# montyhall/bot7

Hardware: AMD Instinct MI355X
Metric: EI candidates scored/sec at N=2048,d=32 (higher is better)
Workload: dtype f64

## Files before the change

bot7_amd/build.py:

```python
import concurrent.futures
import os
import subprocess
import sys

HERE = os.path.dirname(os.path.abspath(__file__))
ROOT = os.path.dirname(HERE)
CSRC = os.path.join(HERE, "csrc")
BUILD = os.path.join(HERE, "_build")
OUT = os.path.join(HERE, "libbot7hip.so")
SOURCES = ["context.hip", "grid_api.hip", "gp_api.hip", "nominate.hip", "blr_api.hip", "sobol.hip", "covar.hip", "potrf.hip", "potrf_persist.hip", "posterior.hip", "score.hip", "extras.hip", "comm.hip", "group.hip", "blr_small.hip", "gp_small.hip", "kpost_small.hip", "batch.hip", "mes.hip", "rff.hip", "slice.hip", "refine.hip", "kg.hip", "ehvi.hip", "trust_region.hip", "ehvi3.hip", "blr_ts.hip", "ts_hvi.hip", "ts_feas.hip", "ts_refine.hip"]
DIAG_ONLY_SOURCES = ["nll_small.hip"]
DIAG_OUT = os.path.join(ROOT, "tools", "_build", "libbot7hip_diag.so")
HEADERS = [os.path.join(CSRC, "b7_internal.h"), os.path.join(CSRC, "gemm_f64.h"), os.path.join(CSRC, "potrf_diag.h"), os.path.join(CSRC, "comm_rccl.h"), os.path.join(CSRC, "ksx_exp.h"), os.path.join(CSRC, "ksx_walk.h"), os.path.join(CSRC, "exp_table.h"), os.path.join(CSRC, "mes_math.h"), os.path.join(CSRC, "logei_math.h"), os.path.join(CSRC, "ehvi_math.h"), os.path.join(CSRC, "counter_rng.h"), os.path.join(CSRC, "gp_small_body.h"), os.path.join(CSRC, "post_ring_layout.h"),
           os.path.join(ROOT, "include", "bot7hip.h")]
HIPCC = os.environ.get("HIPCC", "/opt/rocm/bin/hipcc")
FLAGS = ["-O3", "-std=c++17", "-fPIC", "--offload-arch=gfx950", "-fno-fast-math", "-Wall",
         "-I" + os.path.join(ROOT, "include"), "-I" + CSRC, "-I/opt/rocm/include"]


def _stale(target, deps):
    if not os.path.exists(target):
        return True
    t = os.path.getmtime(target)
    return any(os.path.getmtime(d) > t for d in deps)


EXTRA_FLAGS = {"covar.hip": ["-mllvm", "-amdgpu-mfma-vgpr-form"], "batch.hip": ["-mllvm", "-amdgpu-mfma-vgpr-form"],
               "rff.hip": ["-mllvm", "-amdgpu-mfma-vgpr-form"],
               "ts_refine.hip": ["-mllvm", "-amdgpu-mfma-vgpr-form"],
               "kg.hip": ["-mllvm", "-amdgpu-mfma-vgpr-form"],
               "slice.hip": ["-mllvm", "-disable-machine-licm"]}


def _compile(src, diag=False):
    obj = os.path.join(BUILD, ("diag_" if diag else "") + src.replace(".hip", ".o"))
    path = os.path.join(CSRC, src)
    if _stale(obj, [path] + HEADERS + [os.path.abspath(__file__)]):
        subprocess.check_call([HIPCC] + FLAGS + EXTRA_FLAGS.get(src, []) + (["-DB7_DIAG"] if diag else []) + ["-c", path, "-o", obj])
        return obj, True
    return obj, False


def _mentions_diag(src):
    return "B7_DIAG" in open(os.path.join(CSRC, src)).read()


def build_diag(verbose=False):
    build()
    os.makedirs(os.path.dirname(DIAG_OUT), exist_ok=True)
    todo = [s for s in SOURCES if _mentions_diag(s)] + DIAG_ONLY_SOURCES
    with concurrent.futures.ThreadPoolExecutor(max_workers=min(8, len(todo))) as ex:
        res = dict(zip(todo, ex.map(lambda s: _compile(s, True), todo)))
    objs = [res[s][0] if s in res else os.path.join(BUILD, s.replace(".hip", ".o")) for s in SOURCES + DIAG_ONLY_SOURCES]
    if any(ch for _, ch in res.values()) or _stale(DIAG_OUT, objs):
        subprocess.check_call([HIPCC, "-shared", "-fPIC", "--offload-arch=gfx950", "-o", DIAG_OUT] + objs +
                              ["-ldl", "-Wl,-rpath,/opt/rocm/lib", "-Wl,--no-undefined", "-Wl,-Bsymbolic"])
        if verbose:
            print("built", DIAG_OUT)
    return DIAG_OUT


def posterior_isa():
    out = os.path.join(BUILD, "posterior.s")
    path = os.path.join(CSRC, "posterior.hip")
    if _stale(out, [path] + HEADERS + [os.path.abspath(__file__)]):
        subprocess.check_call([HIPCC] + [f for f in FLAGS if f != "-fPIC"] + ["-S", "--cuda-device-only", "-Wno-unused-command-line-argument",
                                                                            path, "-o", out])
    return out


def check_agpr_discipline():
    import re
    text = open(posterior_isa()).read()
    found = {}
    for m in re.finditer(r"^(_ZN\S*post_kernel_w4(?:ILi(\d)E|tILi\d+ELi\d+E)\S*):[^\n]*\n(.*?)\n\s*s_endpgm", text, flags=re.S | re.M):
        nj = int(m.group(2)) if m.group(2) else 16
        ntiles = 32 if nj == 16 else 8 * nj
        in_asm, stats, bad = False, {"mfma": 0, "mfma_from_zero": 0, "acc_reads": 0, "scratch": 0}, []
        for line in m.group(3).split("\n"):
            code = line.split(";")[0]
            if "ASMSTART" in line:
                in_asm = True
                continue
            if "ASMEND" in line:
                in_asm = False
                continue
            if in_asm:
                stats["mfma"] += "v_mfma_f64_16x16x4_f64" in code
                stats["mfma_from_zero"] += bool(re.search(r"v_mfma_f64_16x16x4_f64 a\[[^\]]*\], v\[[^\]]*\], v\[[^\]]*\], 0\s*$", code))
                stats["acc_reads"] += "v_accvgpr_read_b32" in code
            else:
                if re.search(r"(?<![A-Za-z0-9_.])a(\[|\d)", code):
                    bad.append(line.strip())
                if nj == 16 and re.search(r"\bm0\b", code):
                    bad.append(line.strip())
                stats["scratch"] += "scratch_" in code
        if bad or stats["scratch"] or stats["mfma_from_zero"] != ntiles or stats["acc_reads"] != 8 * ntiles:
            raise RuntimeError("post_kernel_w4<%d>: AGPR discipline broken: %r, compiler-generated AGPR uses: %r"
                               % (nj, stats, bad[:5]))
        found[nj] = stats
    if not {2, 4} <= set(found):
        raise RuntimeError("post_kernel_w4<2> and <4> expected in the ISA of posterior.hip, found %r" % sorted(found))
    return found


def build_post_probe():
    src = os.path.join(ROOT, "tools", "post_probe.hip")
    out = os.path.join(ROOT, "tools", "_build", "post_probe")
    os.makedirs(os.path.dirname(out), exist_ok=True)
    if _stale(out, [src, os.path.join(ROOT, "tools", "post_kernel_w8.h"), os.path.join(CSRC, "posterior.hip")] + HEADERS):
        subprocess.check_call([HIPCC, "--offload-arch=gfx950", "-O3", "-std=c++17", "-fno-fast-math", "-Wno-unused-value",
                               "-DB7_POST_NO_LAUNCHERS", "-I" + os.path.join(ROOT, "include"), "-I" + CSRC,
                               "-I/opt/rocm/include", "-o", out, src, "-Wl,-rpath,/opt/rocm/lib"])
    return out


def build(force=False, verbose=False):
    os.makedirs(BUILD, exist_ok=True)
    if force:
        for f in os.listdir(BUILD):
            os.remove(os.path.join(BUILD, f))
    with concurrent.futures.ThreadPoolExecutor(max_workers=min(8, len(SOURCES) + 2)) as ex:
        isa = ex.submit(check_agpr_discipline)
        probe = ex.submit(build_post_probe)
        results = list(ex.map(_compile, SOURCES))
        isa.result()
        probe.result()
    objs = [o for o, _ in results]
    if any(changed for _, changed in results) or _stale(OUT, objs):
        subprocess.check_call([HIPCC, "-shared", "-fPIC", "--offload-arch=gfx950", "-o", OUT] + objs +
                              ["-ldl", "-Wl,-rpath,/opt/rocm/lib", "-Wl,--no-undefined", "-Wl,-Bsymbolic"])
        if verbose:
            print("built", OUT)
    return OUT

# ... 6 lines not shown
```

bot7_amd/csrc/b7_internal.h:

```cpp
#pragma once
#include <hip/hip_runtime.h>
#include <stddef.h>
#include <stdint.h>

#include <map>
#include <string>
#include <vector>

#include "bot7hip.h"

constexpr int B7_NPAD = 128;
constexpr int B7_PANEL = 64;
constexpr int B7_PERSIST_NMAX = 4096;
constexpr int B7_MROWS = 256;
constexpr int B7_MAX_D = 96;

constexpr int B7_TAB_VAL = 0;
constexpr int B7_TAB_IDX = 1;
constexpr int B7_TAB_STATUS = 2;
constexpr int B7_TAB_ROWS = 3;
constexpr int B7_TAB_ROW0 = 4;
constexpr int B7_TAB_W = B7_TAB_ROW0 + B7_MAX_D;
constexpr int B7_MAX_WORLD = 64;

// ... 105 lines not shown
  double amp = 0, noise = 0, mean = 0;
  b7_gp_opts opts;
  int kernel = B7_KERNEL_ARDSE;
  DevBuf xobs;
  DevBuf w;
  DevBuf zsc;
  DevBuf zss;
  DevBuf K;
  DevBuf L;
  DevBuf Linv;
  DevBuf W;
  DevBuf dinv;
  DevBuf alpha;
  DevBuf resid;
  DevBuf atmp;
  DevBuf info;
  DevBuf ybuf;

  bool predicted = false;
  int64_t Mpred = 0;
  DevBuf mu;
  DevBuf var;
  DevBuf acc;
  bool acc_valid = false;
  int spin_us = 500;
  bool npad_small = true;
  bool potrf_small = true;
  bool blr_small = true;
  double fmin_scalar = 0.0;
  bool acc_fresh = false;
  int acc_kind = 0;
  DevBuf ks;
  size_t ks_bytes = (size_t)4 << 30;
  int diag_variant = 1;
  int inverse_inline = 1;
  PinnedBlock *pinned = nullptr, *pinned_dev = nullptr;
  std::vector<double> net_host;
  PinBuf pin_blr;
  PinBuf pin_eval;
  PinBuf pin_nll;
  PinBuf pin_slice;
  DevBuf slice_state;
  DevBuf slice_trace;
  int slice_trace_rpc = 0;
  int slice_trace_C = 0, slice_trace_D = 0;
  bool fmin_staged = false;
  bool potrf_attrs_set = false;
  bool linv_done = false;
  int potrf_sched = 3;
  int syrk_small = 1;
  int potrf_defer = 1;
  int potrf_group = 2;
  struct JobList { DevBuf buf; int n = 0; };
  std::map<int, JobList> pjobs_cache;
  DevBuf pstamps;
  int pjobs_nb = 0, pjobs_n = 0;
  DevBuf bhyp, bw, bzsc, bzss, bK, bL, bdinv, bflags, binfo, bresid, bterms, bLinv, balpha, bmu, bvar;
  bool persist_attr_set = false, persist_stamps = false;
  int persist_helpers = 0;
  int persist_aborts = 0;
  int nll_small = 1;
  bool kpost_small = true;
  bool fit_small = true;
  int persist_fault = -1;
  int potrf_sched_saved = 0;
  DevBuf part;
// ... 434 lines not shown
```

bot7_amd/csrc/context.hip:

```cpp
#include <stdarg.h>
#include <stdio.h>
#include <stdlib.h>
#include <string.h>

#include "b7_internal.h"

static thread_local std::string g_create_err;

int b7_fail(b7_ctx *c, int code, const char *fmt, ...) {
  char buf[512];
  va_list ap;
  va_start(ap, fmt);
  vsnprintf(buf, sizeof(buf), fmt, ap);
  va_end(ap);
  if (c)
    c->err = buf;
  else
    g_create_err = buf;
  return code;
}

int b7_ensure(b7_ctx *c, DevBuf &b, size_t bytes) {
  if (bytes == 0) bytes = 16;
  if (b.cap >= bytes) return B7_OK;
// ... 133 lines not shown
  if (const char *pv = getenv("B7_TS_FEAS_ONEPASS")) c->ts_feas_onepass = atoi(pv) ? 1 : 0;
#endif
  e = hipStreamCreateWithFlags(&c->stream, hipStreamNonBlocking);
  if (e == hipSuccess) e = hipEventCreateWithFlags(&c->ev_fit, hipEventDisableTiming);
  if (e == hipSuccess) e = hipHostMalloc((void **)&c->pinned, B7_PINNED_BYTES, hipHostMallocMapped);
  if (e == hipSuccess) e = hipHostGetDevicePointer((void **)&c->pinned_dev, c->pinned, 0);
  if (e != hipSuccess) {
    if (c->pinned) (void)hipHostFree(c->pinned);
    if (c->stream) (void)hipStreamDestroy(c->stream);
    delete c;
    return b7_fail(nullptr, B7_ERR_HIP, "stream / pinned result block creation: %s", hipGetErrorString(e));
  }
  if (b7_ensure(c, c->scratch, B7_SCRATCH_BYTES) != B7_OK) {
    g_create_err = c->err;
    b7_destroy(c);
    return B7_ERR_NOMEM;
  }
  *out = c;
  return B7_OK;
}

void b7_destroy(b7_ctx *c) {
  if (!c) return;
  (void)hipSetDevice(c->device);
  (void)hipStreamSynchronize(c->stream);
  (void)b7_comm_destroy(c);
  DevBuf *all[] = {&c->grid[0], &c->grid[1], &c->xobs, &c->w,     &c->zsc,  &c->zss,     &c->K,      &c->L,
                   &c->Linv,    &c->W,       &c->dinv, &c->alpha, &c->resid, &c->info,   &c->ybuf,   &c->mu,
                   &c->var,     &c->acc,     &c->ks,   &c->part,  &c->scratch, &c->tmpgrid, &c->tmpmu, &c->tmpvar, &c->fant, &c->feat, &c->netbuf, &c->atmp, &c->slots, &c->pstamps,
                   &c->bhyp, &c->bw, &c->bzsc, &c->bzss, &c->bK, &c->bL, &c->bdinv, &c->bflags, &c->binfo, &c->bresid, &c->bterms,
                   &c->bLinv, &c->balpha, &c->bmu, &c->bvar, &c->ticket, &c->bel, &c->belvec, &c->ystar, &c->mes_ticket, &c->mes_user,
                   &c->ts_paths, &c->ts_draw, &c->ts_work, &c->ts_user, &c->ts_ref_ws, &c->ts_ref_trace, &c->ts_ref_user, &c->slice_trace, &c->slice_state, &c->refine_ws, &c->refine_trace, &c->refine_user,
                   &c->feas, &c->feas_stage, &c->kg, &c->kgvec, &c->kg_slopes, &c->kg_user,
                   &c->ts_hvi, &c->ts_hvi_t, &c->ts_hvi_user, &c->ts_feas, &c->ts_feas_user, &c->post, &c->ehvi_front, &c->ehvi_user, &c->ehvi3_front, &c->ehvi3_table, &c->ehvi3_user};
  for (auto &kv : c->pjobs_cache) b7_release(kv.second.buf);
  for (DevBuf *b : all) b7_release(*b);
  if (c->tev_init)
    for (int i = 0; i < B7_MAX_TIMERS; ++i) {
      (void)hipEventDestroy(c->tev[i][0]);
      (void)hipEventDestroy(c->tev[i][1]);
    }
  resolve_phases(c);
  if (c->pinned) (void)hipHostFree(c->pinned);
  for (PinBuf *b : {&c->pin_eval, &c->pin_blr, &c->pin_nll, &c->pin_bel, &c->pin_slice, &c->pin_kg})
    if (b->host) (void)hipHostFree(b->host);
  if (c->tab_host) (void)hipHostFree(c->tab_host);
  for (hipEvent_t e : c->free_events) (void)hipEventDestroy(e);
  if (c->phase_e0) (void)hipEventDestroy(c->phase_e0);
  if (c->ev_fit) (void)hipEventDestroy(c->ev_fit);
  for (hipEvent_t e : c->ev_feas)
    if (e) (void)hipEventDestroy(e);
  for (hipEvent_t e : c->ev_ehvi)
    if (e) (void)hipEventDestroy(e);
  for (hipEvent_t e : c->ev_ts_feas)
    if (e) (void)hipEventDestroy(e);
  (void)hipStreamDestroy(c->stream);
  delete c;
}

const char *b7_last_error(const b7_ctx *c) { return c ? c->err.c_str() : g_create_err.c_str(); }

int b7_device_info(b7_ctx *c, char *name_out, int *compute_units, int64_t *hbm_bytes) {
  if (!c) return B7_ERR_INVALID;
  hipDeviceProp_t prop;
  B7_HIP(c, hipGetDeviceProperties(&prop, c->device));
  if (name_out) snprintf(name_out, 64, "%s (%s)", prop.name, prop.gcnArchName);
  if (compute_units) *compute_units = prop.multiProcessorCount;
// ... 62 lines not shown
```

bot7_amd/csrc/posterior.hip:

```cpp
#include "b7_internal.h"
#include "post_ring_layout.h"
#include <utility>

#ifdef B7_POST_STAMPS
__device__ unsigned long long b7_post_stamps[4 * 4096];
extern "C" int b7dbg_post_stamps(unsigned long long *out, int nblocks) {
  return (int)hipMemcpyFromSymbol(out, HIP_SYMBOL(b7_post_stamps), sizeof(unsigned long long) * 4 * nblocks);
}
#endif

typedef double d2_t __attribute__((ext_vector_type(2)));

struct PostBatch {
  int64_t sLinv = 0, sks = 0, svar = 0;
  const double *base = nullptr, *var_add = nullptr;
};

namespace w4 {
constexpr int BM = 128, BK = 16, LD = BK + 1, A_DBL = BM * LD;

#define B7_W4_ACC_REGS \
  "a0", "a1", "a2", "a3", "a4", "a5", "a6", "a7", "a8", "a9", "a10", "a11", "a12", "a13", "a14", "a15", \
  "a16", "a17", "a18", "a19", "a20", "a21", "a22", "a23", "a24", "a25", "a26", "a27", "a28", "a29", "a30", \
  "a31", "a32", "a33", "a34", "a35", "a36", "a37", "a38", "a39", "a40", "a41", "a42", "a43", "a44", "a45", \
  "a46", "a47", "a48", "a49", "a50", "a51", "a52", "a53", "a54", "a55", "a56", "a57", "a58", "a59", "a60", \
  "a61", "a62", "a63", "a64", "a65", "a66", "a67", "a68", "a69", "a70", "a71", "a72", "a73", "a74", "a75", \
  "a76", "a77", "a78", "a79", "a80", "a81", "a82", "a83", "a84", "a85", "a86", "a87", "a88", "a89", "a90", \
  "a91", "a92", "a93", "a94", "a95", "a96", "a97", "a98", "a99", "a100", "a101", "a102", "a103", "a104", \
  "a105", "a106", "a107", "a108", "a109", "a110", "a111", "a112", "a113", "a114", "a115", "a116", "a117", \
  "a118", "a119", "a120", "a121", "a122", "a123", "a124", "a125", "a126", "a127", "a128", "a129", "a130", \
  "a131", "a132", "a133", "a134", "a135", "a136", "a137", "a138", "a139", "a140", "a141", "a142", "a143", \
  "a144", "a145", "a146", "a147", "a148", "a149", "a150", "a151", "a152", "a153", "a154", "a155", "a156", \
  "a157", "a158", "a159", "a160", "a161", "a162", "a163", "a164", "a165", "a166", "a167", "a168", "a169", \
  "a170", "a171", "a172", "a173", "a174", "a175", "a176", "a177", "a178", "a179", "a180", "a181", "a182", \
  "a183", "a184", "a185", "a186", "a187", "a188", "a189", "a190", "a191", "a192", "a193", "a194", "a195", \
  "a196", "a197", "a198", "a199", "a200", "a201", "a202", "a203", "a204", "a205", "a206", "a207", "a208", \
  "a209", "a210", "a211", "a212", "a213", "a214", "a215", "a216", "a217", "a218", "a219", "a220", "a221", \
  "a222", "a223", "a224", "a225", "a226", "a227", "a228", "a229", "a230", "a231", "a232", "a233", "a234", \
  "a235", "a236", "a237", "a238", "a239", "a240", "a241", "a242", "a243", "a244", "a245", "a246", "a247", \
  "a248", "a249", "a250", "a251", "a252", "a253", "a254", "a255"
// ... 182 lines not shown
      constexpr int h = decltype(hj_)::value / NJ, j = decltype(hj_)::value % NJ;
      double s = 0.0;
      static_for<4>([&](auto i_) {
        double v[4];
        read_tile<NJ, 4 * h + decltype(i_)::value, j>(v);
#pragma unroll
        for (int r = 0; r < 4; ++r) s = __builtin_fma(v[r], v[r], s);
      });
      colss[h][j] += s;
    });
  }
#undef B7_STAGE

#pragma unroll
  for (int j = 0; j < NJ; ++j) {
    double v0 = colss[0][j], v1 = colss[1][j];
    v0 += __shfl_xor(v0, 16);
    v0 += __shfl_xor(v0, 32);
    v1 += __shfl_xor(v1, 16);
    v1 += __shfl_xor(v1, 32);
    const int64_t gidx = row0 + (int64_t)blockIdx.x * BN + wave * 16 * NJ + j * 16 + lane;
    if (lane < 16 && gidx < Mtotal) {
      double ss = v0;
      ss += v1;
      double v = (base + sgn * ss) + var_add;
      if (clamp) v = (v < var_min) ? var_min : v;
      var[gidx] = v;
    }
  }
#ifdef B7_POST_STAMPS
  if (threadIdx.x == 0 && blockIdx.x < 4096) {
    const unsigned long long st1 = __builtin_amdgcn_s_memtime(), sr1 = __builtin_amdgcn_s_memrealtime();
    __builtin_amdgcn_s_waitcnt(0xC07F);
    unsigned long long *o = b7_post_stamps + 4 * blockIdx.x;
    o[0] = st0, o[1] = sr0, o[2] = st1, o[3] = sr1;
  }
#endif
}

template <int NJ>
constexpr int lds_bytes() { return 2 * (BM + 64 * NJ) * LD * 8; }

template <int NJ, int NR>
struct Tall {
  static constexpr int BMT = 16 * NR, BN = 64 * NJ, ROWS = BMT + BN;
  static constexpr int STAGE_BYTES = ROWS * post_ring::ROW_BYTES, NBUF = 3;
  static constexpr int ND = ROWS / post_ring::PIECE_ROWS / post_ring::WAVES;
  static constexpr int NDA = BMT / post_ring::PIECE_ROWS / post_ring::WAVES;
  static constexpr int NP = NR + NJ;
  static constexpr int LDS_BYTES = NBUF * STAGE_BYTES;
  static_assert(NJ * NR == 32, "32 accumulator tiles per wave");
  static_assert(ND == 12 && ND % 3 == 0, "vmcnt(12) below is ND; a third of the pieces per k-step");
  static_assert(LDS_BYTES <= 160 * 1024, "three stage images in 160 KiB");

  struct Set {
    double a[NR], b[NJ];
  };
  typedef __attribute__((address_space(3))) double lds_double;
  struct Lane {
    int fa[NBUF][4], fb[NBUF][4];
    unsigned src, dst[NBUF];
    __device__ __forceinline__ void rotate1() {
#pragma unroll
      for (int s = 0; s < 4; ++s) {
        const int a = fa[0][s], b = fb[0][s];
        fa[0][s] = fa[1][s], fa[1][s] = fa[2][s], fa[2][s] = a;
        fb[0][s] = fb[1][s], fb[1][s] = fb[2][s], fb[2][s] = b;
      }
// ... 52 lines not shown
    int n = 0;
    for (int d = 0; d < H; ++d) n += (d + 1) * NS / (H + 1) < x;
    return n;
  }
  static constexpr bool is_dma(int x) { return dma_before(x + 1) > dma_before(x); }

  template <int FIRST, int NEXT_FIRST, bool ZERO, int POS>
  static __device__ __forceinline__ void stage(Set &s0, Set &s1, const Lane &ln,
                                               const char *__restrict__ pa, const char *__restrict__ pb, int64_t lda, Cursor &ld) {
    constexpr int CUR = POS % NBUF, NXT = (POS + 1) % NBUF, DST = (POS + 2) % NBUF;
    const int64_t step = 32 * lda * 8;
    const char *ga = pa + (((int64_t)ld.t * BMT) * lda + ld.kb * BK) * 8, *gb = pb + (int64_t)(ld.kb * BK) * 8;
    ld.advance();
    auto sides = [&](auto ks_, Set &into, auto x_) {
      constexpr int ks = decltype(ks_)::value, x = decltype(x_)::value, r = x - dma_before(x);
      if constexpr (is_dma(x))
        dma_piece<H * ks + dma_before(x)>(ga, gb, step, ln.src, ln.dst[DST]);
      else if constexpr (r < NJ || r - NJ >= FIRST)
        read_one<r, ks + 1, CUR>(into, ln);
    };
    kstep<FIRST, ZERO, NS, 0>(s0, [&](auto x_) { sides(std::integral_constant<int, 0>{}, s1, x_); });
    kstep<FIRST, false, NS, 0>(s1, [&](auto x_) { sides(std::integral_constant<int, 1>{}, s0, x_); });
    kstep<FIRST, false, NS, 3>(s0, [&](auto x_) { sides(std::integral_constant<int, 2>{}, s1, x_); });
    asm volatile("s_waitcnt vmcnt(12) lgkmcnt(0)" ::: "memory");
    __builtin_amdgcn_s_barrier();
    kstep<FIRST, false, NP, 0>(s1, [&](auto s_) {
      constexpr int x = decltype(s_)::value;
      if constexpr (x < NJ || x - NJ >= NEXT_FIRST) read_one<x, 0, NXT>(s0, ln);
    });
  }
};

template <int NJ, int NR>
__global__ void __launch_bounds__(256)
    post_kernel_w4t(const double *__restrict__ Linv, const double *__restrict__ ks, int Npad, int64_t row0, int64_t Mtotal,
                    double base, double sgn, double var_add, int clamp, double var_min, double *__restrict__ var,
                    PostBatch bat) {
  using T = Tall<NJ, NR>;
  constexpr int BMT = T::BMT, BN = T::BN, NP = T::NP;
  extern __shared__ __align__(16) double sm[];
  if (bat.base) {
    const int64_t y = blockIdx.y;
    Linv += y * bat.sLinv;
    ks += y * bat.sks;
    var += y * bat.svar;
    base = bat.base[y];
    if (bat.var_add) var_add = bat.var_add[y];
  }
  const int lane = threadIdx.x & 63, wave = __builtin_amdgcn_readfirstlane(threadIdx.x >> 6);
#ifdef B7_POST_STAMPS
  const unsigned long long st0 = __builtin_amdgcn_s_memtime(), sr0 = __builtin_amdgcn_s_memrealtime();
  __builtin_amdgcn_s_waitcnt(0xC07F);
#endif
  const int64_t lda = Npad;
  const char *pa = reinterpret_cast<const char *>(Linv + (int64_t)(post_ring::PIECE_ROWS * wave) * lda);
  const char *pb = reinterpret_cast<const char *>(ks + ((int64_t)blockIdx.x * BN + post_ring::PIECE_ROWS * wave) * lda);
  typename T::Lane ln;
  {
    const post_ring::Chunk c = post_ring::dma_src(wave, lane);
    ln.src = (unsigned)(((c.row - post_ring::PIECE_ROWS * wave) * Npad + 2 * c.chunk) * 8);
  }
  const unsigned lds0 = (unsigned)(uintptr_t)(__attribute__((address_space(3))) void *)sm;
#pragma unroll
  for (int b = 0; b < T::NBUF; ++b) {
#pragma unroll
    for (int s = 0; s < 4; ++s) {
      ln.fa[b][s] = lds0 + b * T::STAGE_BYTES + post_ring::frag_byte(lane & 15, 4 * s + (lane >> 4));
      ln.fb[b][s] = ln.fa[b][s] + (BMT + wave * 16 * NJ) * post_ring::ROW_BYTES;
      asm volatile("" : "+v"(ln.fa[b][s]), "+v"(ln.fb[b][s]));
    }
    ln.dst[b] = lds0 + b * T::STAGE_BYTES + wave * post_ring::PIECE_BYTES;
  }

  const int ntiles = Npad / BMT;
  typename T::Cursor ld{0, 0, ntiles};
  typename T::Set s0, s1;
  {
    const int64_t step = 32 * lda * 8;
    static_for<T::ND>([&](auto c_) { T::template dma_piece<decltype(c_)::value>(pa, pb, step, ln.src, ln.dst[0]); });
    ld.advance();
    const char *ga = pa + (((int64_t)ld.t * BMT) * lda + ld.kb * BK) * 8, *gb = pb + (int64_t)(ld.kb * BK) * 8;
    static_for<T::ND>([&](auto c_) { T::template dma_piece<decltype(c_)::value>(ga, gb, step, ln.src, ln.dst[1]); });
    ld.advance();
  }
  asm volatile("s_waitcnt vmcnt(12)" ::: "memory");
  __builtin_amdgcn_s_barrier();
  static_for<NP>([&](auto p_) { T::template read_one<decltype(p_)::value, 0, 0>(s0, ln); });

  double colss[2][NJ] = {};
#define B7_STAGE(F, NF, Z, POS) T::template stage<F, NF, Z, POS>(s0, s1, ln, pa, pb, lda, ld)
  for (int t = 0; t < ntiles; ++t) {
    B7_STAGE(0, 0, true, 0);
    if (t > 0) {
      const int n = NR * t - 1;
      for (int p = 0; p < n / 3; ++p) {
        B7_STAGE(0, 0, false, 1);
        B7_STAGE(0, 0, false, 2);
        B7_STAGE(0, 0, false, 0);
      }
      if (n % 3 >= 1) B7_STAGE(0, 0, false, 1);
      if (n % 3 == 2) B7_STAGE(0, 0, false, 2);
      ln.rotate((n + 1) % 3);
      B7_STAGE(0, 1, false, 0);
    }
    static_for<NR - 1>([&](auto q_) {
      constexpr int Q = decltype(q_)::value + 1;
      B7_STAGE(Q, (Q + 1) % NR, false, Q % 3);
    });
    ln.rotate(NR % 3);
    asm volatile("s_nop 15\n\ts_nop 15\n\ts_nop 15" ::: "memory");
    static_for<(NR / 4) * NJ>([&](auto qj_) {
      constexpr int q = decltype(qj_)::value / NJ, j = decltype(qj_)::value % NJ;
      double s = 0.0;
      static_for<4>([&](auto i_) {
        double v[4];
        read_tile<NJ, 4 * q + decltype(i_)::value, j>(v);
#pragma unroll
        for (int r = 0; r < 4; ++r) s = __builtin_fma(v[r], v[r], s);
      });
      colss[q & 1][j] += s;
    });
  }
#undef B7_STAGE
  asm volatile("s_waitcnt vmcnt(0)" ::: "memory");

#pragma unroll
  for (int j = 0; j < NJ; ++j) {
    double v0 = colss[0][j], v1 = colss[1][j];
    v0 += __shfl_xor(v0, 16);
    v0 += __shfl_xor(v0, 32);
    v1 += __shfl_xor(v1, 16);
    v1 += __shfl_xor(v1, 32);
    const int64_t gidx = row0 + (int64_t)blockIdx.x * BN + wave * 16 * NJ + j * 16 + lane;
    if (lane < 16 && gidx < Mtotal) {
      double ss = v0;
      ss += v1;
      double v = (base + sgn * ss) + var_add;
      if (clamp) v = (v < var_min) ? var_min : v;
      var[gidx] = v;
    }
  }
#ifdef B7_POST_STAMPS
  if (threadIdx.x == 0 && blockIdx.x < 4096) {
    const unsigned long long st1 = __builtin_amdgcn_s_memtime(), sr1 = __builtin_amdgcn_s_memrealtime();
    __builtin_amdgcn_s_waitcnt(0xC07F);
    unsigned long long *o = b7_post_stamps + 4 * blockIdx.x;
    o[0] = st0, o[1] = sr0, o[2] = st1, o[3] = sr1;
  }
#endif
}
}

namespace small64 {
typedef double d4_t __attribute__((ext_vector_type(4)));
constexpr int NB = 64, LLD = NB + 2, BN = 64;
constexpr int LDS_BYTES = BN * LLD * 8;

__global__ void __launch_bounds__(256)
    post_small_kernel(const double *__restrict__ Linv, const double *__restrict__ ks, int64_t row0, int64_t Mtotal, int ntiles,
                      double base, double sgn, double var_add, int clamp, double var_min, double *__restrict__ var, PostBatch bat) {
  extern __shared__ __align__(16) double sm[];
  if (bat.base) {
    const int64_t y = blockIdx.y;
    Linv += y * bat.sLinv;
    ks += y * bat.sks;
    var += y * bat.svar;
    base = bat.base[y];
    if (bat.var_add) var_add = bat.var_add[y];
  }
  double *Ks = sm;
  const int tid = threadIdx.x, lane = tid & 63, wave = tid >> 6, lr = lane & 15, lq = lane >> 4;
  d2_t pv[BN / 8];
  auto fetch = [&](int tile) {
    const double *kt = ks + ((int64_t)tile * BN) * NB;
#pragma unroll
    for (int i = 0; i < BN / 8; ++i) {
      const int e = tid + 256 * i;
      pv[i] = *reinterpret_cast<const d2_t *>(kt + (int64_t)(e >> 5) * NB + 2 * (e & 31));
    }
  };
  int tile = blockIdx.x;
  if (tile < ntiles) fetch(tile);
// ... 59 lines not shown
#ifndef B7_POST_NO_LAUNCHERS
namespace {
struct PostArgs {
  const double *Linv, *ks;
  double *var;
  double base, sgn, var_add;
  int S;
  PostBatch pb;
};

template <int NJ>
int launch_post_w4(b7_ctx *c, const PostArgs &a, int64_t row0, int64_t rows, int64_t Mtotal) {
  constexpr int lds = w4::lds_bytes<NJ>();
  B7_HIP(c, hipFuncSetAttribute(reinterpret_cast<const void *>(w4::post_kernel_w4<NJ>),
                                hipFuncAttributeMaxDynamicSharedMemorySize, lds));
  hipLaunchKernelGGL(w4::post_kernel_w4<NJ>, dim3((unsigned)(rows / (64 * NJ)), a.S), dim3(256), lds, c->stream, a.Linv, a.ks,
                     c->Npad, row0, Mtotal, a.base, a.sgn, a.var_add, c->opts.var_clamp, c->opts.var_min, a.var, a.pb);
  B7_HIP(c, hipGetLastError());
  return B7_OK;
}

template <int NJ, int NR>
int launch_post_tall(b7_ctx *c, const PostArgs &a, int64_t row0, int64_t rows, int64_t Mtotal) {
  using T = w4::Tall<NJ, NR>;
  auto kern = w4::post_kernel_w4t<NJ, NR>;
  B7_HIP(c, hipFuncSetAttribute(reinterpret_cast<const void *>(kern), hipFuncAttributeMaxDynamicSharedMemorySize,
                                T::LDS_BYTES));
  hipLaunchKernelGGL(kern, dim3((unsigned)(rows / T::BN), a.S), dim3(256), T::LDS_BYTES, c->stream, a.Linv, a.ks, c->Npad, row0,
                     Mtotal, a.base, a.sgn, a.var_add, c->opts.var_clamp, c->opts.var_min, a.var, a.pb);
  B7_HIP(c, hipGetLastError());
  return B7_OK;
}

int launch_post_small(b7_ctx *c, const PostArgs &a, int64_t row0, int64_t rows, int64_t Mtotal) {
  B7_HIP(c, hipFuncSetAttribute(reinterpret_cast<const void *>(small64::post_small_kernel), hipFuncAttributeMaxDynamicSharedMemorySize,
                                small64::LDS_BYTES));
  const int ntiles = (int)(rows / small64::BN), S = a.S > 0 ? a.S : 1;
  int gx = (2 * c->cus + S - 1) / S;
  if (gx > ntiles) gx = ntiles;
  if (gx < 1) gx = 1;
  hipLaunchKernelGGL(small64::post_small_kernel, dim3((unsigned)gx, S), dim3(256), small64::LDS_BYTES, c->stream, a.Linv, a.ks, row0,
                     Mtotal, ntiles, a.base, a.sgn, a.var_add, c->opts.var_clamp, c->opts.var_min, a.var, a.pb);
  B7_HIP(c, hipGetLastError());
  return B7_OK;
}

int dispatch_post(b7_ctx *c, const PostArgs &a, int64_t row0, int64_t rows, int64_t Mtotal) {
  if (rows % B7_MROWS) return b7_fail(c, B7_ERR_INVALID, "post: rows %lld not a multiple of %d", (long long)rows, B7_MROWS);
  if (c->Npad == 64) return launch_post_small(c, a, row0, rows, Mtotal);
  const bool large = rows / 256 * a.S >= c->cus;
  if (c->Npad % 256 == 0 && large) return launch_post_tall<2, 16>(c, a, row0, rows, Mtotal);
  if (!large) return launch_post_w4<2>(c, a, row0, rows, Mtotal);
  return launch_post_w4<4>(c, a, row0, rows, Mtotal);
}
}

int launch_post(b7_ctx *c, const FitSet &f, const double *ks, int64_t row0, int64_t rows, int64_t Mtotal, double *var) {
  PhaseScope ps(c, "post");
  const bool blr = c->model_kind == 1;
  PostArgs a{f.Linv, ks, var, blr ? 0.0 : f.amp, blr ? 1.0 : -1.0, blr ? f.noise : (c->opts.var_with_noise ? f.noise : 0.0), 1,
             PostBatch{}};
  return dispatch_post(c, a, row0, rows, Mtotal);
}

int launch_post_batch(b7_ctx *c, const FitSet &f, const double *ks, int64_t sks, int64_t rows, int64_t Mtotal, double *var,
                      int64_t svar) {
  PhaseScope ps(c, "post");
  PostArgs a{f.Linv, ks, var, 0.0, -1.0, 0.0, f.S, PostBatch{}};
  a.pb.sLinv = FitSet::s_Linv(c->Npad, c->dpad);
  a.pb.sks = sks;
  a.pb.svar = svar;
  a.pb.base = f.amp_dev;
  a.pb.var_add = c->opts.var_with_noise ? f.noise_dev : nullptr;
  return dispatch_post(c, a, 0, rows, Mtotal);
}

int launch_post_heads(b7_ctx *c, int S, const double *Linv, const double *feat, int64_t rows, int64_t Mtotal, double *var, int64_t svar,
                      const double *zero_dev, const double *invbeta_dev) {
  PhaseScope ps(c, "post");
  PostArgs a{Linv, feat, var, 0.0, 1.0, 0.0, S, PostBatch{}};
  a.pb.sLinv = FitSet::s_Linv(c->Npad, c->dpad);
  a.pb.sks = 0;
  a.pb.svar = svar;
  a.pb.base = zero_dev;
// ... 5 lines not shown
```

Measured before the change: 16.45 million.

## Run tall posterior variance through a persistent atomic work queue with split-K tail

Replaces the one-block-per-tile tall posterior kernel with a persistent kernel, one block per CU, that pulls work items from a global atomic counter. The aim is to remove tail imbalance when the tile count does not divide evenly across CUs. The last tiles can be split along the K dimension into per-slot partial sums, and a separate combine kernel reduces those partials. The cost is an atomic per item, a memset, and possibly an extra kernel launch and partial-sum traffic. With the default split depth of 1, only up to CU-count tiles are split, and only when more than one K tile exists.

```diff
diff --git a/bot7_amd/build.py b/bot7_amd/build.py
--- a/bot7_amd/build.py
+++ b/bot7_amd/build.py
@@ -11,7 +11,7 @@
 SOURCES = ["context.hip", "grid_api.hip", "gp_api.hip", "nominate.hip", "blr_api.hip", "sobol.hip", "covar.hip", "potrf.hip", "potrf_persist.hip", "posterior.hip", "score.hip", "extras.hip", "comm.hip", "group.hip", "blr_small.hip", "gp_small.hip", "kpost_small.hip", "batch.hip", "mes.hip", "rff.hip", "slice.hip", "refine.hip", "kg.hip", "ehvi.hip", "trust_region.hip", "ehvi3.hip", "blr_ts.hip", "ts_hvi.hip", "ts_feas.hip", "ts_refine.hip"]
 DIAG_ONLY_SOURCES = ["nll_small.hip"]
 DIAG_OUT = os.path.join(ROOT, "tools", "_build", "libbot7hip_diag.so")
-HEADERS = [os.path.join(CSRC, "b7_internal.h"), os.path.join(CSRC, "gemm_f64.h"), os.path.join(CSRC, "potrf_diag.h"), os.path.join(CSRC, "comm_rccl.h"), os.path.join(CSRC, "ksx_exp.h"), os.path.join(CSRC, "ksx_walk.h"), os.path.join(CSRC, "exp_table.h"), os.path.join(CSRC, "mes_math.h"), os.path.join(CSRC, "logei_math.h"), os.path.join(CSRC, "ehvi_math.h"), os.path.join(CSRC, "counter_rng.h"), os.path.join(CSRC, "gp_small_body.h"), os.path.join(CSRC, "post_ring_layout.h"),
+HEADERS = [os.path.join(CSRC, "b7_internal.h"), os.path.join(CSRC, "gemm_f64.h"), os.path.join(CSRC, "potrf_diag.h"), os.path.join(CSRC, "comm_rccl.h"), os.path.join(CSRC, "ksx_exp.h"), os.path.join(CSRC, "ksx_walk.h"), os.path.join(CSRC, "exp_table.h"), os.path.join(CSRC, "mes_math.h"), os.path.join(CSRC, "logei_math.h"), os.path.join(CSRC, "ehvi_math.h"), os.path.join(CSRC, "counter_rng.h"), os.path.join(CSRC, "gp_small_body.h"), os.path.join(CSRC, "post_ring_layout.h"), os.path.join(CSRC, "post_queue_sched.h"),
            os.path.join(ROOT, "include", "bot7hip.h")]
 HIPCC = os.environ.get("HIPCC", "/opt/rocm/bin/hipcc")
 FLAGS = ["-O3", "-std=c++17", "-fPIC", "--offload-arch=gfx950", "-fno-fast-math", "-Wall",
@@ -73,7 +73,7 @@
     import re
     text = open(posterior_isa()).read()
     found = {}
-    for m in re.finditer(r"^(_ZN\S*post_kernel_w4(?:ILi(\d)E|tILi\d+ELi\d+E)\S*):[^\n]*\n(.*?)\n\s*s_endpgm", text, flags=re.S | re.M):
+    for m in re.finditer(r"^(_ZN\S*post_kernel_w4(?:ILi(\d)E|qILi\d+ELi\d+E)\S*):[^\n]*\n(.*?)\n\s*s_endpgm", text, flags=re.S | re.M):
         nj = int(m.group(2)) if m.group(2) else 16
         ntiles = 32 if nj == 16 else 8 * nj
         in_asm, stats, bad = False, {"mfma": 0, "mfma_from_zero": 0, "acc_reads": 0, "scratch": 0}, []
@@ -99,8 +99,8 @@
             raise RuntimeError("post_kernel_w4<%d>: AGPR discipline broken: %r, compiler-generated AGPR uses: %r"
                                % (nj, stats, bad[:5]))
         found[nj] = stats
-    if not {2, 4} <= set(found):
-        raise RuntimeError("post_kernel_w4<2> and <4> expected in the ISA of posterior.hip, found %r" % sorted(found))
+    if not {2, 4, 16} <= set(found):
+        raise RuntimeError("post_kernel_w4<2>, <4> and the tall shape's queue kernel expected in the ISA of posterior.hip, found %r" % sorted(found))
     return found
 
 
diff --git a/bot7_amd/csrc/b7_internal.h b/bot7_amd/csrc/b7_internal.h
--- a/bot7_amd/csrc/b7_internal.h
+++ b/bot7_amd/csrc/b7_internal.h
@@ -161,6 +161,7 @@
   int acc_kind = 0;
   DevBuf ks;
   size_t ks_bytes = (size_t)4 << 30;
+  DevBuf postq;
   int diag_variant = 1;
   int inverse_inline = 1;
   PinnedBlock *pinned = nullptr, *pinned_dev = nullptr;
diff --git a/bot7_amd/csrc/context.hip b/bot7_amd/csrc/context.hip
--- a/bot7_amd/csrc/context.hip
+++ b/bot7_amd/csrc/context.hip
@@ -189,7 +189,7 @@
                    &c->bLinv, &c->balpha, &c->bmu, &c->bvar, &c->ticket, &c->bel, &c->belvec, &c->ystar, &c->mes_ticket, &c->mes_user,
                    &c->ts_paths, &c->ts_draw, &c->ts_work, &c->ts_user, &c->ts_ref_ws, &c->ts_ref_trace, &c->ts_ref_user, &c->slice_trace, &c->slice_state, &c->refine_ws, &c->refine_trace, &c->refine_user,
                    &c->feas, &c->feas_stage, &c->kg, &c->kgvec, &c->kg_slopes, &c->kg_user,
-                   &c->ts_hvi, &c->ts_hvi_t, &c->ts_hvi_user, &c->ts_feas, &c->ts_feas_user, &c->post, &c->ehvi_front, &c->ehvi_user, &c->ehvi3_front, &c->ehvi3_table, &c->ehvi3_user};
+                   &c->ts_hvi, &c->ts_hvi_t, &c->ts_hvi_user, &c->ts_feas, &c->ts_feas_user, &c->post, &c->postq,&c->ehvi_front, &c->ehvi_user, &c->ehvi3_front, &c->ehvi3_table, &c->ehvi3_user};
   for (auto &kv : c->pjobs_cache) b7_release(kv.second.buf);
   for (DevBuf *b : all) b7_release(*b);
   if (c->tev_init)
diff --git a/bot7_amd/csrc/post_queue_sched.h b/bot7_amd/csrc/post_queue_sched.h
--- /dev/null
+++ b/bot7_amd/csrc/post_queue_sched.h
@@ -0,0 +1,28 @@
+#pragma once
+
+namespace post_queue {
+#ifndef B7_POST_SPLIT_DEPTH
+#define B7_POST_SPLIT_DEPTH 1
+#endif
+constexpr int SPLIT_DEPTH = B7_POST_SPLIT_DEPTH;
+
+struct Sched {
+  int C, F, T, S, W, items;
+};
+struct Item {
+  int fit, tile, t0, t1, slot;
+};
+
+constexpr int part_doubles(int NJ, int NR) { return NR / 4 * NJ * 256; }
+
+constexpr Sched make(int C, int F, int T, int G, int R) {
+  const int tiles = C * F, S = T == 1 ? 0 : (tiles < R * G ? tiles : R * G);
+  return Sched{C, F, T, S, tiles - S, tiles - S + S * T};
+}
+
+constexpr Item decode(const Sched &s, int i) {
+  if (i < s.W) return Item{i / s.C, i % s.C, 0, s.T, -1};
+  const int k = i - s.W, t = s.T - 1 - k / s.S, slot = k % s.S, u = s.W + slot;
+  return Item{u / s.C, u % s.C, t, t + 1, slot};
+}
+}
diff --git a/bot7_amd/csrc/posterior.hip b/bot7_amd/csrc/posterior.hip
--- a/bot7_amd/csrc/posterior.hip
+++ b/bot7_amd/csrc/posterior.hip
@@ -1,11 +1,18 @@
 #include "b7_internal.h"
 #include "post_ring_layout.h"
+#include "post_queue_sched.h"
+#include <cstdlib>
+#include <cstring>
 #include <utility>
 
 #ifdef B7_POST_STAMPS
-__device__ unsigned long long b7_post_stamps[4 * 4096];
+__device__ unsigned long long b7_post_stamps[5 * 4096];
 extern "C" int b7dbg_post_stamps(unsigned long long *out, int nblocks) {
-  return (int)hipMemcpyFromSymbol(out, HIP_SYMBOL(b7_post_stamps), sizeof(unsigned long long) * 4 * nblocks);
+  return (int)hipMemcpyFromSymbol(out, HIP_SYMBOL(b7_post_stamps), sizeof(unsigned long long) * 5 * nblocks);
+}
+__device__ __forceinline__ unsigned long long b7_post_where() {
+  const unsigned long long xcc = __builtin_amdgcn_s_getreg(20 | (31 << 11)), hw = __builtin_amdgcn_s_getreg(4 | (31 << 11));
+  return xcc << 32 | hw;
 }
 #endif
 
@@ -254,8 +261,8 @@
   if (threadIdx.x == 0 && blockIdx.x < 4096) {
     const unsigned long long st1 = __builtin_amdgcn_s_memtime(), sr1 = __builtin_amdgcn_s_memrealtime();
     __builtin_amdgcn_s_waitcnt(0xC07F);
-    unsigned long long *o = b7_post_stamps + 4 * blockIdx.x;
-    o[0] = st0, o[1] = sr0, o[2] = st1, o[3] = sr1;
+    unsigned long long *o = b7_post_stamps + 5 * blockIdx.x;
+    o[0] = st0, o[1] = sr0, o[2] = st1, o[3] = sr1, o[4] = b7_post_where();
   }
 #endif
 }
@@ -374,52 +381,36 @@
 };
 
 template <int NJ, int NR>
-__global__ void __launch_bounds__(256)
-    post_kernel_w4t(const double *__restrict__ Linv, const double *__restrict__ ks, int Npad, int64_t row0, int64_t Mtotal,
-                    double base, double sgn, double var_add, int clamp, double var_min, double *__restrict__ var,
-                    PostBatch bat) {
+__device__ __forceinline__ void tall_lane(typename Tall<NJ, NR>::Lane &ln, const double *sm, int lane, int wave, int Npad) {
   using T = Tall<NJ, NR>;
-  constexpr int BMT = T::BMT, BN = T::BN, NP = T::NP;
-  extern __shared__ __align__(16) double sm[];
-  if (bat.base) {
-    const int64_t y = blockIdx.y;
-    Linv += y * bat.sLinv;
-    ks += y * bat.sks;
-    var += y * bat.svar;
-    base = bat.base[y];
-    if (bat.var_add) var_add = bat.var_add[y];
-  }
-  const int lane = threadIdx.x & 63, wave = __builtin_amdgcn_readfirstlane(threadIdx.x >> 6);
-#ifdef B7_POST_STAMPS
-  const unsigned long long st0 = __builtin_amdgcn_s_memtime(), sr0 = __builtin_amdgcn_s_memrealtime();
-  __builtin_amdgcn_s_waitcnt(0xC07F);
-#endif
-  const int64_t lda = Npad;
-  const char *pa = reinterpret_cast<const char *>(Linv + (int64_t)(post_ring::PIECE_ROWS * wave) * lda);
-  const char *pb = reinterpret_cast<const char *>(ks + ((int64_t)blockIdx.x * BN + post_ring::PIECE_ROWS * wave) * lda);
-  typename T::Lane ln;
   {
     const post_ring::Chunk c = post_ring::dma_src(wave, lane);
     ln.src = (unsigned)(((c.row - post_ring::PIECE_ROWS * wave) * Npad + 2 * c.chunk) * 8);
   }
-  const unsigned lds0 = (unsigned)(uintptr_t)(__attribute__((address_space(3))) void *)sm;
+  const unsigned lds0 = (unsigned)(uintptr_t)(__attribute__((address_space(3))) const void *)sm;
 #pragma unroll
   for (int b = 0; b < T::NBUF; ++b) {
 #pragma unroll
     for (int s = 0; s < 4; ++s) {
       ln.fa[b][s] = lds0 + b * T::STAGE_BYTES + post_ring::frag_byte(lane & 15, 4 * s + (lane >> 4));
-      ln.fb[b][s] = ln.fa[b][s] + (BMT + wave * 16 * NJ) * post_ring::ROW_BYTES;
+      ln.fb[b][s] = ln.fa[b][s] + (T::BMT + wave * 16 * NJ) * post_ring::ROW_BYTES;
       asm volatile("" : "+v"(ln.fa[b][s]), "+v"(ln.fb[b][s]));
     }
     ln.dst[b] = lds0 + b * T::STAGE_BYTES + wave * post_ring::PIECE_BYTES;
   }
-
-  const int ntiles = Npad / BMT;
-  typename T::Cursor ld{0, 0, ntiles};
+}
+
+template <int NJ, int NR>
+__device__ __forceinline__ void tall_item(typename Tall<NJ, NR>::Lane &ln, const char *__restrict__ pa, const char *__restrict__ pb,
+                                          int64_t lda, int t0, int t1, double *__restrict__ part, double (&colss)[2][NJ]) {
+  using T = Tall<NJ, NR>;
+  constexpr int BMT = T::BMT, NP = T::NP;
+  typename T::Cursor ld{t0, 0, t1};
   typename T::Set s0, s1;
   {
     const int64_t step = 32 * lda * 8;
-    static_for<T::ND>([&](auto c_) { T::template dma_piece<decltype(c_)::value>(pa, pb, step, ln.src, ln.dst[0]); });
+    const char *g0 = pa + ((int64_t)ld.t * BMT) * lda * 8;
+    static_for<T::ND>([&](auto c_) { T::template dma_piece<decltype(c_)::value>(g0, pb, step, ln.src, ln.dst[0]); });
     ld.advance();
     const char *ga = pa + (((int64_t)ld.t * BMT) * lda + ld.kb * BK) * 8, *gb = pb + (int64_t)(ld.kb * BK) * 8;
     static_for<T::ND>([&](auto c_) { T::template dma_piece<decltype(c_)::value>(ga, gb, step, ln.src, ln.dst[1]); });
@@ -429,9 +420,8 @@
   __builtin_amdgcn_s_barrier();
   static_for<NP>([&](auto p_) { T::template read_one<decltype(p_)::value, 0, 0>(s0, ln); });
 
-  double colss[2][NJ] = {};
 #define B7_STAGE(F, NF, Z, POS) T::template stage<F, NF, Z, POS>(s0, s1, ln, pa, pb, lda, ld)
-  for (int t = 0; t < ntiles; ++t) {
+  for (int t = t0; t < t1; ++t) {
     B7_STAGE(0, 0, true, 0);
     if (t > 0) {
       const int n = NR * t - 1;
@@ -460,12 +450,20 @@
 #pragma unroll
         for (int r = 0; r < 4; ++r) s = __builtin_fma(v[r], v[r], s);
       });
-      colss[q & 1][j] += s;
+      if (part)
+        part[(q * NJ + j) * 256 + threadIdx.x] = s;
+      else
+        colss[q & 1][j] += s;
     });
   }
 #undef B7_STAGE
-  asm volatile("s_waitcnt vmcnt(0)" ::: "memory");
-
+  asm volatile("s_waitcnt vmcnt(0) lgkmcnt(0)" ::: "memory");
+}
+
+template <int NJ>
+__device__ __forceinline__ void tall_epilogue(const double (&colss)[2][NJ], int64_t cand0, int64_t Mtotal, int lane, int wave,
+                                              double base, double sgn, double var_add, int clamp, double var_min,
+                                              double *__restrict__ var) {
 #pragma unroll
   for (int j = 0; j < NJ; ++j) {
     double v0 = colss[0][j], v1 = colss[1][j];
@@ -473,7 +471,7 @@
     v0 += __shfl_xor(v0, 32);
     v1 += __shfl_xor(v1, 16);
     v1 += __shfl_xor(v1, 32);
-    const int64_t gidx = row0 + (int64_t)blockIdx.x * BN + wave * 16 * NJ + j * 16 + lane;
+    const int64_t gidx = cand0 + wave * 16 * NJ + j * 16 + lane;
     if (lane < 16 && gidx < Mtotal) {
       double ss = v0;
       ss += v1;
@@ -482,14 +480,114 @@
       var[gidx] = v;
     }
   }
+}
+
 #ifdef B7_POST_STAMPS
-  if (threadIdx.x == 0 && blockIdx.x < 4096) {
-    const unsigned long long st1 = __builtin_amdgcn_s_memtime(), sr1 = __builtin_amdgcn_s_memrealtime();
-    __builtin_amdgcn_s_waitcnt(0xC07F);
-    unsigned long long *o = b7_post_stamps + 4 * blockIdx.x;
-    o[0] = st0, o[1] = sr0, o[2] = st1, o[3] = sr1;
-  }
+#define B7_POST_STAMP_BEGIN \
+  const unsigned long long st0 = __builtin_amdgcn_s_memtime(), sr0 = __builtin_amdgcn_s_memrealtime(); \
+  __builtin_amdgcn_s_waitcnt(0xC07F);
+#define B7_POST_STAMP_END(EXTRA) \
+  if (threadIdx.x == 0 && blockIdx.y == 0 && blockIdx.x < 4096) { \
+    const unsigned long long st1 = __builtin_amdgcn_s_memtime(), sr1 = __builtin_amdgcn_s_memrealtime(); \
+    __builtin_amdgcn_s_waitcnt(0xC07F); \
+    unsigned long long *o = b7_post_stamps + 5 * blockIdx.x; \
+    o[0] = st0, o[1] = sr0, o[2] = st1, o[3] = sr1, o[4] = b7_post_where() | (unsigned long long)(EXTRA) << 40; \
+  }
+#else
+#define B7_POST_STAMP_BEGIN
+#define B7_POST_STAMP_END(EXTRA)
 #endif
+
+template <int NJ, int NR>
+__global__ void __launch_bounds__(256)
+    post_kernel_w4t(const double *__restrict__ Linv, const double *__restrict__ ks, int Npad, int64_t row0, int64_t Mtotal,
+                    double base, double sgn, double var_add, int clamp, double var_min, double *__restrict__ var,
+                    PostBatch bat) {
+  using T = Tall<NJ, NR>;
+  extern __shared__ __align__(16) double sm[];
+  if (bat.base) {
+    const int64_t y = blockIdx.y;
+    Linv += y * bat.sLinv;
+    ks += y * bat.sks;
+    var += y * bat.svar;
+    base = bat.base[y];
+    if (bat.var_add) var_add = bat.var_add[y];
+  }
+  const int lane = threadIdx.x & 63, wave = __builtin_amdgcn_readfirstlane(threadIdx.x >> 6);
+  B7_POST_STAMP_BEGIN
+  const int64_t lda = Npad;
+  const char *pa = reinterpret_cast<const char *>(Linv + (int64_t)(post_ring::PIECE_ROWS * wave) * lda);
+  const char *pb = reinterpret_cast<const char *>(ks + ((int64_t)blockIdx.x * T::BN + post_ring::PIECE_ROWS * wave) * lda);
+  typename T::Lane ln;
+  tall_lane<NJ, NR>(ln, sm, lane, wave, Npad);
+  double colss[2][NJ] = {};
+  tall_item<NJ, NR>(ln, pa, pb, lda, 0, Npad / T::BMT, nullptr, colss);
+  tall_epilogue<NJ>(colss, row0 + (int64_t)blockIdx.x * T::BN, Mtotal, lane, wave, base, sgn, var_add, clamp, var_min, var);
+  B7_POST_STAMP_END(1)
+}
+
+template <int NJ, int NR>
+__global__ void __launch_bounds__(256)
+    post_kernel_w4q(const double *__restrict__ Linv, const double *__restrict__ ks, int Npad, int64_t row0, int64_t Mtotal,
+                    double base, double sgn, double var_add, int clamp, double var_min, double *__restrict__ var,
+                    PostBatch bat, post_queue::Sched sch, unsigned *__restrict__ counter, double *__restrict__ parts) {
+  using T = Tall<NJ, NR>;
+  extern __shared__ __align__(16) double sm[];
+  int *const word = reinterpret_cast<int *>(reinterpret_cast<char *>(sm) + T::LDS_BYTES);
+  const int lane = threadIdx.x & 63, wave = __builtin_amdgcn_readfirstlane(threadIdx.x >> 6);
+  B7_POST_STAMP_BEGIN
+  const int64_t lda = Npad;
+  typename T::Lane ln;
+  tall_lane<NJ, NR>(ln, sm, lane, wave, Npad);
+  [[maybe_unused]] int taken = 0;
+  for (;;) {
+    if (threadIdx.x == 0) *word = (int)__hip_atomic_fetch_add(counter, 1u, __ATOMIC_RELAXED, __HIP_MEMORY_SCOPE_AGENT);
+    __syncthreads();
+    const int i = __builtin_amdgcn_readfirstlane(*word);
+    if (i >= sch.items) break;
+    ++taken;
+    const post_queue::Item it = post_queue::decode(sch, i);
+    const double *Li = Linv, *ki = ks;
+    if (bat.base) {
+      Li += it.fit * bat.sLinv;
+      ki += it.fit * bat.sks;
+    }
+    const char *pa = reinterpret_cast<const char *>(Li + (int64_t)(post_ring::PIECE_ROWS * wave) * lda);
+    const char *pb = reinterpret_cast<const char *>(ki + ((int64_t)it.tile * T::BN + post_ring::PIECE_ROWS * wave) * lda);
+    double colss[2][NJ] = {};
+    double *part = it.slot < 0 ? nullptr : parts + ((int64_t)it.slot * sch.T + it.t0) * post_queue::part_doubles(NJ, NR);
+    tall_item<NJ, NR>(ln, pa, pb, lda, it.t0, it.t1, part, colss);
+    if (it.slot < 0) {
+      double b = base, va = var_add, *vi = var;
+      if (bat.base) {
+        vi += it.fit * bat.svar;
+        b = bat.base[it.fit];
+        if (bat.var_add) va = bat.var_add[it.fit];
+      }
+      tall_epilogue<NJ>(colss, row0 + (int64_t)it.tile * T::BN, Mtotal, lane, wave, b, sgn, va, clamp, var_min, vi);
+    }
+  }
+  B7_POST_STAMP_END(taken)
+}
+
+template <int NJ, int NR>
+__global__ void __launch_bounds__(256)
+    post_combine_kernel(const double *__restrict__ parts, post_queue::Sched sch, int64_t row0, int64_t Mtotal, double base, double sgn,
+                        double var_add, int clamp, double var_min, double *__restrict__ var, PostBatch bat) {
+  constexpr int NQ = NR / 4;
+  const int lane = threadIdx.x & 63, wave = __builtin_amdgcn_readfirstlane(threadIdx.x >> 6);
+  const int u = sch.W + blockIdx.x, fit = u / sch.C, tile = u % sch.C;
+  if (bat.base) {
+    var += fit * bat.svar;
+    base = bat.base[fit];
+    if (bat.var_add) var_add = bat.var_add[fit];
+  }
+  const double *p = parts + (int64_t)blockIdx.x * sch.T * post_queue::part_doubles(NJ, NR) + threadIdx.x;
+  double colss[2][NJ] = {};
+  for (int t = 0; t < sch.T; ++t, p += post_queue::part_doubles(NJ, NR))
+#pragma unroll
+    for (int qj = 0; qj < NQ * NJ; ++qj) colss[(qj / NJ) & 1][qj % NJ] += p[qj * 256];
+  tall_epilogue<NJ>(colss, row0 + (int64_t)tile * Tall<NJ, NR>::BN, Mtotal, lane, wave, base, sgn, var_add, clamp, var_min, var);
 }
 }
 
@@ -615,6 +713,31 @@
   return B7_OK;
 }
 
+template <int NJ, int NR>
+int launch_post_queue(b7_ctx *c, const PostArgs &a, int64_t row0, int64_t rows, int64_t Mtotal) {
+  using T = w4::Tall<NJ, NR>;
+  constexpr size_t HEAD = 256;
+  constexpr int LDS = T::LDS_BYTES + 16;
+  static_assert(LDS <= 160 * 1024, "ring + item word in 160 KiB");
+  const int ntiles = c->Npad / T::BMT;
+  const post_queue::Sched sch = post_queue::make((int)(rows / T::BN), a.S, ntiles, c->cus, post_queue::SPLIT_DEPTH);
+  B7_TRY(b7_ensure(c, c->postq, HEAD + sizeof(double) * post_queue::part_doubles(NJ, NR) * (size_t)ntiles * post_queue::SPLIT_DEPTH * c->cus));
+  unsigned *counter = static_cast<unsigned *>(c->postq.p);
+  double *parts = reinterpret_cast<double *>(static_cast<char *>(c->postq.p) + HEAD);
+  auto kern = w4::post_kernel_w4q<NJ, NR>;
+  B7_HIP(c, hipFuncSetAttribute(reinterpret_cast<const void *>(kern), hipFuncAttributeMaxDynamicSharedMemorySize, LDS));
+  B7_HIP(c, hipMemsetAsync(counter, 0, sizeof(unsigned), c->stream));
+  hipLaunchKernelGGL(kern, dim3((unsigned)(sch.items < c->cus ? sch.items : c->cus)), dim3(256), LDS, c->stream, a.Linv, a.ks, c->Npad,
+                     row0, Mtotal, a.base, a.sgn, a.var_add, c->opts.var_clamp, c->opts.var_min, a.var, a.pb, sch, counter, parts);
+  B7_HIP(c, hipGetLastError());
+  if (sch.S) {
+    hipLaunchKernelGGL((w4::post_combine_kernel<NJ, NR>), dim3((unsigned)sch.S), dim3(256), 0, c->stream, parts, sch, row0, Mtotal,
+                       a.base, a.sgn, a.var_add, c->opts.var_clamp, c->opts.var_min, a.var, a.pb);
+    B7_HIP(c, hipGetLastError());
+  }
+  return B7_OK;
+}
+
 int launch_post_small(b7_ctx *c, const PostArgs &a, int64_t row0, int64_t rows, int64_t Mtotal) {
   B7_HIP(c, hipFuncSetAttribute(reinterpret_cast<const void *>(small64::post_small_kernel), hipFuncAttributeMaxDynamicSharedMemorySize,
                                 small64::LDS_BYTES));
@@ -632,7 +755,13 @@
   if (rows % B7_MROWS) return b7_fail(c, B7_ERR_INVALID, "post: rows %lld not a multiple of %d", (long long)rows, B7_MROWS);
   if (c->Npad == 64) return launch_post_small(c, a, row0, rows, Mtotal);
   const bool large = rows / 256 * a.S >= c->cus;
-  if (c->Npad % 256 == 0 && large) return launch_post_tall<2, 16>(c, a, row0, rows, Mtotal);
+#if defined(B7_DIAG) || defined(B7_POST_STAMPS)
+  if (const char *pv = getenv("B7_POST_QUEUE")) {
+    if (c->Npad % 256 == 0 && large && atoi(pv) == 0) return launch_post_tall<2, 16>(c, a, row0, rows, Mtotal);
+    if (c->Npad % 256 == 0 && atoi(pv) == 2) return launch_post_queue<2, 16>(c, a, row0, rows, Mtotal);
+  }
+#endif
+  if (c->Npad % 256 == 0 && large) return launch_post_queue<2, 16>(c, a, row0, rows, Mtotal);
   if (!large) return launch_post_w4<2>(c, a, row0, rows, Mtotal);
   return launch_post_w4<4>(c, a, row0, rows, Mtotal);
 }
```

New measurement: 16.59 million (median of 6 runs). About the same (+0.9%).
